# ErickRosete/tacorl

Measured on NVIDIA B200. Metric: play_lmp_train_frames_per_sec, higher is better.
Workload: dtype bf16

## Files before the change

tacorl_b200/csrc/gemm_tc.cu:

```cuda
#include "common.cuh"
#include "internal.h"
#include <cuda.h>
#include <cuda_bf16.h>
#include <algorithm>

namespace tacorl {

constexpr int TC_BM = 128;
constexpr int TC_BK = 64;
constexpr int TC_UMMA_K = 16;
constexpr int TC_THREADS = 192;

__device__ __forceinline__ uint32_t smem_u32(const void* p) { return (uint32_t)__cvta_generic_to_shared(p); }

__device__ __forceinline__ void mbar_init(uint32_t bar, uint32_t count) {
  asm volatile("mbarrier.init.shared::cta.b64 [%0], %1;" ::"r"(bar), "r"(count));
}
__device__ __forceinline__ void mbar_expect_tx(uint32_t bar, uint32_t bytes) {
  asm volatile("mbarrier.arrive.expect_tx.shared::cta.b64 _, [%0], %1;" ::"r"(bar), "r"(bytes) : "memory");
}
__device__ __forceinline__ void mbar_wait(uint32_t bar, uint32_t parity) {
  uint32_t done;
  do {
    asm volatile(
// ... 501 lines not shown
    for (int j = 0; j < 4; ++j) {
      if (ep.act == ACT_RELU) v[j] = fmaxf(v[j], 0.f);
      else if (ep.act == ACT_SILU) v[j] = v[j] / (1.f + __expf(-v[j]));
      if (g4[j] <= 0.f) v[j] = 0.f;
    }
    if (ep.C) *reinterpret_cast<float4*>(ep.C + (long long)b * ep.ldc + col) = make_float4(v[0], v[1], v[2], v[3]);
    if (ep.Cb) {
      __nv_bfloat162 lo = __floats2bfloat162_rn(v[0], v[1]), hi = __floats2bfloat162_rn(v[2], v[3]);
      uint2 pk = make_uint2(*reinterpret_cast<uint32_t*>(&lo), *reinterpret_cast<uint32_t*>(&hi));
      *reinterpret_cast<uint2*>(ep.Cb + (long long)b * ep.ldcb + col) = pk;
    }
  }
  RS_STAMP(9)
#ifdef RS_EXP_LATEARRIVE
  asm volatile("barrier.cluster.arrive.release.aligned;" ::: "memory");
#endif
  asm volatile("barrier.cluster.wait.aligned;" ::: "memory");
  RS_STAMP(10)
  RS_STAMP(11)
  RS_CTA_STAMP(1)
}

struct SeqArgs {
  int n_steps;
  int tau0, dtau;
  float beta;
  float* C; long long ldc, c_ts;
  const float* gate; long long ldgate, gate_ts;
  __nv_bfloat16* Cb; long long cb_ts;
  int act;
  unsigned* flags;
};
__device__ unsigned g_rnn_seq_timeouts = 0;
__device__ unsigned g_rnn_flags[2][32];
__device__ unsigned g_rnn_done = 0;
__device__ __forceinline__ void rnn_launch_epilogue(int tid) {
  if (tid == 0) {
    __threadfence();
    const unsigned total = gridDim.x * gridDim.y * gridDim.z;
    if (atomicAdd(&g_rnn_done, 1u) == total - 1) {
#pragma unroll
      for (int i = 0; i < 64; ++i) (&g_rnn_flags[0][0])[i] = 0;
      __threadfence();
      g_rnn_done = 0;
    }
  }
}
#ifdef TACORL_STEP_PROFILE
__device__ long long g_seq_prof[16];
#define SQ_STAMP(i) if (step == 8 && blockIdx.x == 1 && blockIdx.y == 3) g_seq_prof[i] = clock64();
#else
#define SQ_STAMP(i)
#endif

__device__ __forceinline__ void tma_load_3d(uint32_t dst, const CUtensorMap* tm, int c0, int c1, int c2, uint32_t bar) {
  asm volatile(
      "cp.async.bulk.tensor.3d.shared::cluster.global.mbarrier::complete_tx::bytes [%0], [%1, {%2, %3, %4}], [%5];"
      ::"r"(dst), "l"(tm), "r"(c0), "r"(c1), "r"(c2), "r"(bar) : "memory");
}
__device__ __forceinline__ unsigned ld_acquire_gpu(const unsigned* p) {
  unsigned v;
  asm volatile("ld.acquire.gpu.global.u32 %0, [%1];" : "=r"(v) : "l"(p) : "memory");
  return v;
}
__device__ __forceinline__ void red_release_gpu_add(unsigned* p, unsigned v) {
  asm volatile("red.release.gpu.global.add.u32 [%0], %1;" ::"l"(p), "r"(v) : "memory");
}

__global__ void __cluster_dims__(RS_KS, 1, 1) __launch_bounds__(RS_THREADS, 1)
rnn_seq_kernel(const __grid_constant__ CUtensorMap tmA, const __grid_constant__ CUtensorMap tmW, const SeqArgs sa,
               int M, int Mpad, int N, int NT, int kb_per_cta) {
  extern __shared__ __align__(1024) uint8_t smem_raw[];
  uint8_t* smem = (uint8_t*)(((uintptr_t)smem_raw + 1023) & ~(uintptr_t)1023);
  const uint32_t A_TILE = 128 * 128, W_BYTES = (uint32_t)NT * 128, W_STAGE = (W_BYTES + 1023) & ~1023u;
  const int SP = NT + 4;
  const int per = Mpad / RS_KS;
  uint8_t* w_smem = smem;
  uint8_t* a_smem = smem + (size_t)kb_per_cta * W_STAGE;
  float* S = (float*)(a_smem + (size_t)kb_per_cta * A_TILE);
  uint64_t* bars = (uint64_t*)((uint8_t*)S + (((size_t)((Mpad + 31) & ~31) * SP * 4 + 1023) & ~(size_t)1023));
  uint32_t* tmem_slot = (uint32_t*)(bars + 10);
  const int tid = threadIdx.x, warp = tid >> 5, lane = tid & 31;
  const uint32_t rank = blockIdx.x;
  const int tile = blockIdx.y, n0 = tile * NT, tiles = gridDim.y;
  const uint32_t tmem_cols = NT <= 32 ? 32 : (NT <= 64 ? 64 : (NT <= 128 ? 128 : 256));
  const uint32_t done_bar = smem_u32(bars + 8), w_bar = smem_u32(bars + 9);

  if (tid == RS_EPI) {
    for (int s = 0; s < kb_per_cta; ++s) mbar_init(smem_u32(bars + s), 1);
    mbar_init(done_bar, 1);
    mbar_init(w_bar, 1);
    asm volatile("fence.mbarrier_init.release.cluster;" ::: "memory");
  }
  if (warp == RS_EPI / 32) {
    asm volatile("tcgen05.alloc.cta_group::1.sync.aligned.shared::cta.b32 [%0], %1;"
                 ::"r"(smem_u32(tmem_slot)), "r"(tmem_cols) : "memory");
    asm volatile("tcgen05.relinquish_alloc_permit.cta_group::1.sync.aligned;" ::: "memory");
  }
  tc_fence_before();
  __syncthreads();
  tc_fence_after();
  const uint32_t tmem_base = *tmem_slot;
  const int k_begin = (int)rank * kb_per_cta * TC_BK;

  if (tid == RS_EPI) {
    mbar_expect_tx(w_bar, (uint32_t)kb_per_cta * W_BYTES);
    for (int s = 0; s < kb_per_cta; ++s)
      tma_load_2d(smem_u32(w_smem + (size_t)s * W_STAGE), &tmW, k_begin + s * TC_BK, n0, w_bar);
  }
  const int j_lo = k_begin / NT, j_hi = min(tiles - 1, (k_begin + kb_per_cta * TC_BK - 1) / NT);
  const int NT4 = NT >> 2, elems = per * NT4;
  bool dead = false;

  for (int step = 0; step < sa.n_steps; ++step) {
    const int tau = sa.tau0 + step * sa.dtau;
// ... 114 lines not shown
#pragma unroll
      for (int i = 0; i < RS_MAXE; ++i) dep += acc[i].x + acc[i].y + acc[i].z + acc[i].w;
      asm volatile("barrier.cluster.arrive.release.aligned;" ::"f"(dep) : "memory");
      if (tid == 0) { SQ_STAMP(8) }
      float* Ct = sa.C + (long long)tau * sa.c_ts;
      __nv_bfloat16* Bt = sa.Cb + (long long)tau * sa.cb_ts;
      float4 outv[RS_MAXE];
      bool okv[RS_MAXE];
#pragma unroll
      for (int i = 0; i < RS_MAXE; ++i) {
        const int e = tid + i * RS_EPI;
        const int bi = e / NT4, n = (e - bi * NT4) * 4, b = (int)rank * per + bi, col = n0 + n;
        okv[i] = e < elems && b < M && col < N;
        float v[4] = {acc[i].x, acc[i].y, acc[i].z, acc[i].w};
        const float c4[4] = {cold[i].x, cold[i].y, cold[i].z, cold[i].w};
        const float g4[4] = {gt[i].x, gt[i].y, gt[i].z, gt[i].w};
#pragma unroll
        for (int j = 0; j < 4; ++j) {
          v[j] = fmaf(sa.beta, c4[j], v[j]);
          if (sa.act == ACT_RELU) v[j] = fmaxf(v[j], 0.f);
          if (g4[j] <= 0.f) v[j] = 0.f;
        }
        outv[i] = make_float4(v[0], v[1], v[2], v[3]);
        if (okv[i]) {
          __nv_bfloat162 lo = __floats2bfloat162_rn(v[0], v[1]), hi = __floats2bfloat162_rn(v[2], v[3]);
          *reinterpret_cast<uint2*>(Bt + (long long)b * N + col) =
              make_uint2(*reinterpret_cast<uint32_t*>(&lo), *reinterpret_cast<uint32_t*>(&hi));
        }
      }
      asm volatile("fence.proxy.async.global;" ::: "memory");
      if (tid == 0) { SQ_STAMP(9) }
      asm volatile("bar.sync 1, %0;" ::"n"(RS_EPI) : "memory");
      if (tid == 0) { __threadfence(); red_release_gpu_add(&g_rnn_flags[0][tile], 1u); SQ_STAMP(10) }
#pragma unroll
      for (int i = 0; i < RS_MAXE; ++i) {
        const int e = tid + i * RS_EPI;
        const int bi = e / NT4, n = (e - bi * NT4) * 4, b = (int)rank * per + bi, col = n0 + n;
        if (okv[i]) *reinterpret_cast<float4*>(Ct + (long long)b * sa.ldc + col) = outv[i];
      }
    } else {
      asm volatile("barrier.cluster.arrive.release.aligned;" ::: "memory");
    }
  }
  asm volatile("barrier.cluster.wait.aligned;" ::: "memory");
  if (warp == RS_EPI / 32) {
    tc_fence_after();
    asm volatile("tcgen05.dealloc.cta_group::1.sync.aligned.b32 %0, %1;" ::"r"(tmem_base), "r"(tmem_cols) : "memory");
  }
  rnn_launch_epilogue(tid);
}

constexpr int RW_KS = 4;
constexpr int RW_MAX_TILES = 16;
struct WaveLane {
  int n_steps, tau0, dtau, act;
  float beta;
  float* C; long long ldc, c_ts;
  const float* gate; long long ldgate, gate_ts;
  __nv_bfloat16* Cb; long long ldcb, cb_ts;
  unsigned* flags;
};
struct WaveArgs { WaveLane lane[2]; };

__global__ void __launch_bounds__(RS_THREADS, 1)
rnn_wave_kernel(const __grid_constant__ CUtensorMap tmA0, const __grid_constant__ CUtensorMap tmW0,
                const __grid_constant__ CUtensorMap tmA1, const __grid_constant__ CUtensorMap tmW1,
                const __grid_constant__ WaveArgs wa, int M, int Mpad, int N, int NT, int kb_per_cta) {
  extern __shared__ __align__(1024) uint8_t smem_raw[];
  uint8_t* smem = (uint8_t*)(((uintptr_t)smem_raw + 1023) & ~(uintptr_t)1023);
  const uint32_t W_BYTES = (uint32_t)NT * 128, W_STAGE = (W_BYTES + 1023) & ~1023u, A_PITCH = (uint32_t)Mpad * 128;
  const int SP = NT + 4;
  const int per = Mpad / RW_KS;
  uint8_t* w_smem = smem;
  uint8_t* a_smem = smem + (size_t)kb_per_cta * W_STAGE;
  float* S = (float*)(a_smem + (size_t)kb_per_cta * A_PITCH);
  uint64_t* bars = (uint64_t*)((uint8_t*)S + (((size_t)((Mpad + 31) & ~31) * SP * 4 + 1023) & ~(size_t)1023));
  uint32_t* tmem_slot = (uint32_t*)(bars + 10);
  const int tid = threadIdx.x, warp = tid >> 5, lane = tid & 31;
  const uint32_t rank = blockIdx.x;
  const int tile = blockIdx.y, n0 = tile * NT, tiles = gridDim.y;
  const WaveLane& sa = wa.lane[blockIdx.z];
  const CUtensorMap* tmA = blockIdx.z ? &tmA1 : &tmA0;
  const CUtensorMap* tmW = blockIdx.z ? &tmW1 : &tmW0;
  const uint32_t tmem_cols = NT <= 32 ? 32 : (NT <= 64 ? 64 : 128);
  const uint32_t done_bar = smem_u32(bars + 8), w_bar = smem_u32(bars + 9);

  if (tid == RS_EPI) {
    for (int s = 0; s < kb_per_cta; ++s) mbar_init(smem_u32(bars + s), 1);
    mbar_init(done_bar, 1);
    mbar_init(w_bar, 1);
    asm volatile("fence.mbarrier_init.release.cluster;" ::: "memory");
  }
  if (warp == RS_EPI / 32) {
    asm volatile("tcgen05.alloc.cta_group::1.sync.aligned.shared::cta.b32 [%0], %1;"
                 ::"r"(smem_u32(tmem_slot)), "r"(tmem_cols) : "memory");
    asm volatile("tcgen05.relinquish_alloc_permit.cta_group::1.sync.aligned;" ::: "memory");
  }
  tc_fence_before();
  __syncthreads();
  tc_fence_after();
  const uint32_t tmem_base = *tmem_slot;
  const int k_begin = (int)rank * kb_per_cta * TC_BK;

  if (tid == RS_EPI) {
    mbar_expect_tx(w_bar, (uint32_t)kb_per_cta * W_BYTES);
    for (int s = 0; s < kb_per_cta; ++s)
      tma_load_2d(smem_u32(w_smem + (size_t)s * W_STAGE), tmW, k_begin + s * TC_BK, n0, w_bar);
  }
  const int j_lo = k_begin / NT, j_hi = min(tiles - 1, (k_begin + kb_per_cta * TC_BK - 1) / NT);
  const int NT4 = NT >> 2, elems = per * NT4;
  bool dead = false;

  for (int step = 0; step < sa.n_steps; ++step) {
    const int tau = sa.tau0 + step * sa.dtau;
    const uint32_t ph = (uint32_t)step & 1u;
    float4 cold[RS_MAXE], gt[RS_MAXE];
    if (warp == RS_EPI / 32) {
      if (step > 0 && !dead) {
        const unsigned want = (unsigned)(RW_KS * step);
        bool bad = false;
        for (int j = j_lo + lane; j <= j_hi; j += 32) {
          unsigned spins = 0;
          while (ld_acquire_gpu(&g_rnn_flags[blockIdx.z][j]) < want) {
            if (++spins > (1u << 21)) { bad = true; atomicAdd(&g_rnn_seq_timeouts, 1u); break; }
          }
        }
        if (__any_sync(0xffffffffu, bad)) dead = true;
        __threadfence();
        __syncwarp();
      }
      if (lane == 0) {
        if (step == 0) mbar_wait(w_bar, 0);
        asm volatile("fence.proxy.async.global;" ::: "memory");
        for (int s = 0; s < kb_per_cta; ++s) {
          const uint32_t bar = smem_u32(bars + s);
          mbar_expect_tx(bar, A_PITCH);
          tma_load_3d(smem_u32(a_smem + (size_t)s * A_PITCH), tmA, k_begin + s * TC_BK, 0, tau - sa.dtau, bar);
        }
        const uint32_t idesc = (1u << 4) | (1u << 7) | (1u << 10) | ((uint32_t)(NT >> 3) << 17) | ((uint32_t)(128 >> 4) << 24);
        for (int s = 0; s < kb_per_cta; ++s) {
          mbar_wait(smem_u32(bars + s), ph);
          tc_fence_after();
          const uint32_t a_src = smem_u32(a_smem + (size_t)s * A_PITCH), w_src = smem_u32(w_smem + (size_t)s * W_STAGE);
#pragma unroll
          for (int k = 0; k < TC_BK / TC_UMMA_K; ++k)
            tc_mma_bf16(tmem_base, make_smem_desc(a_src + k * 32, 16, 1024), make_smem_desc(w_src + k * 32, 16, 1024), idesc,
                        (s > 0 || k > 0) ? 1u : 0u);
        }
        tc_commit(done_bar);
      }
      __syncwarp();
    } else {
      const float* Ct = sa.C + (long long)tau * sa.c_ts;
      const float* Gt = sa.gate ? sa.gate + (long long)tau * sa.gate_ts : nullptr;
      long long offc[RS_MAXE], offg[RS_MAXE];
#pragma unroll
      for (int i = 0; i < RS_MAXE; ++i) {
        const int e = tid + i * RS_EPI;
        const int bi = e / NT4, n = (e - bi * NT4) * 4, b = (int)rank * per + bi, col = n0 + n;
        const bool ok = e < elems && b < M && col < N;
        offc[i] = ok ? (long long)b * sa.ldc + col : 0;
        offg[i] = ok ? (long long)b * sa.ldgate + col : 0;
      }
      const float4 zero = make_float4(0.f, 0.f, 0.f, 0.f), one = make_float4(1.f, 1.f, 1.f, 1.f);
#pragma unroll
      for (int i = 0; i < RS_MAXE; ++i) cold[i] = sa.beta != 0.f ? *reinterpret_cast<const float4*>(Ct + offc[i]) : zero;
#pragma unroll
      for (int i = 0; i < RS_MAXE; ++i) gt[i] = Gt ? *reinterpret_cast<const float4*>(Gt + offg[i]) : one;
      mbar_wait(done_bar, ph);
      tc_fence_after();
    }
    if (step > 0) asm volatile("barrier.cluster.wait.aligned;" ::: "memory");
    if (warp < RS_EPI / 32) {
      const int q = warp & 3;
      if (q * 32 < Mpad) {
        float* Srow = S + (q * 32 + lane) * SP;
        uint32_t r[2][16];
#pragma unroll
        for (int i = 0; i < 2; ++i) {
          const int c0 = (warp >> 2) * 16 + 64 * i;
          if (c0 < NT) tc_ld16_nowait(tmem_base + ((uint32_t)(q * 32) << 16) + c0, r[i]);
        }
        tc_ld_wait();
#pragma unroll
        for (int i = 0; i < 2; ++i) {
          const int c0 = (warp >> 2) * 16 + 64 * i;
          if (c0 < NT) {
#pragma unroll
            for (int j = 0; j < 4; ++j)
              reinterpret_cast<float4*>(Srow + c0)[j] = make_float4(__uint_as_float(r[i][4 * j]), __uint_as_float(r[i][4 * j + 1]),
                                                                    __uint_as_float(r[i][4 * j + 2]), __uint_as_float(r[i][4 * j + 3]));
          }
        }
      }
    }
    tc_fence_before();
    cluster_sync_all();
    tc_fence_after();
    float4 acc[RS_MAXE];
    if (warp < RS_EPI / 32) {
      float4 part[RS_MAXE][RW_KS];
#pragma unroll
      for (int i = 0; i < RS_MAXE; ++i) {
        const int e = tid + i * RS_EPI;
        const int bi = e / NT4, n = (e - bi * NT4) * 4;
        const uint32_t addr = smem_u32(S + ((int)rank * per + (e < elems ? bi : 0)) * SP + (e < elems ? n : 0));
#pragma unroll
        for (int q = 0; q < RW_KS; ++q) part[i][q] = ld_dsmem_v4(addr, (q + rank) & (RW_KS - 1));
      }
#pragma unroll
      for (int i = 0; i < RS_MAXE; ++i) {
        float4 v = make_float4(0.f, 0.f, 0.f, 0.f);
#pragma unroll
        for (int q = 0; q < RW_KS; ++q) { v.x += part[i][q].x; v.y += part[i][q].y; v.z += part[i][q].z; v.w += part[i][q].w; }
        acc[i] = v;
      }
      float dep = 0.f;
#pragma unroll
      for (int i = 0; i < RS_MAXE; ++i) dep += acc[i].x + acc[i].y + acc[i].z + acc[i].w;
      asm volatile("barrier.cluster.arrive.release.aligned;" ::"f"(dep) : "memory");
      float* Ct = sa.C + (long long)tau * sa.c_ts;
      __nv_bfloat16* Bt = sa.Cb + (long long)tau * sa.cb_ts;
      float4 outv[RS_MAXE];
      bool okv[RS_MAXE];
#pragma unroll
      for (int i = 0; i < RS_MAXE; ++i) {
        const int e = tid + i * RS_EPI;
        const int bi = e / NT4, n = (e - bi * NT4) * 4, b = (int)rank * per + bi, col = n0 + n;
        okv[i] = e < elems && b < M && col < N;
        float v[4] = {acc[i].x, acc[i].y, acc[i].z, acc[i].w};
        const float c4[4] = {cold[i].x, cold[i].y, cold[i].z, cold[i].w};
        const float g4[4] = {gt[i].x, gt[i].y, gt[i].z, gt[i].w};
#pragma unroll
        for (int j = 0; j < 4; ++j) {
          v[j] = fmaf(sa.beta, c4[j], v[j]);
          if (sa.act == ACT_RELU) v[j] = fmaxf(v[j], 0.f);
          if (g4[j] <= 0.f) v[j] = 0.f;
        }
        outv[i] = make_float4(v[0], v[1], v[2], v[3]);
        if (okv[i]) {
          __nv_bfloat162 lo = __floats2bfloat162_rn(v[0], v[1]), hi = __floats2bfloat162_rn(v[2], v[3]);
          *reinterpret_cast<uint2*>(Bt + (long long)b * sa.ldcb + col) =
              make_uint2(*reinterpret_cast<uint32_t*>(&lo), *reinterpret_cast<uint32_t*>(&hi));
        }
      }
      asm volatile("fence.proxy.async.global;" ::: "memory");
      asm volatile("bar.sync 1, %0;" ::"n"(RS_EPI) : "memory");
      if (tid == 0) { __threadfence(); red_release_gpu_add(&g_rnn_flags[blockIdx.z][tile], 1u); }
#pragma unroll
      for (int i = 0; i < RS_MAXE; ++i) {
        const int e = tid + i * RS_EPI;
        const int bi = e / NT4, n = (e - bi * NT4) * 4, b = (int)rank * per + bi, col = n0 + n;
        if (okv[i]) *reinterpret_cast<float4*>(Ct + (long long)b * sa.ldc + col) = outv[i];
      }
    } else {
      asm volatile("barrier.cluster.arrive.release.aligned;" ::: "memory");
    }
  }
  if (sa.n_steps > 0) asm volatile("barrier.cluster.wait.aligned;" ::: "memory");
  if (warp == RS_EPI / 32) {
    tc_fence_after();
    asm volatile("tcgen05.dealloc.cta_group::1.sync.aligned.b32 %0, %1;" ::"r"(tmem_base), "r"(tmem_cols) : "memory");
  }
  rnn_launch_epilogue(tid);
}

typedef CUresult (*EncodeTiledFn)(CUtensorMap*, CUtensorMapDataType, cuuint32_t, void*, const cuuint64_t*,
                                  const cuuint64_t*, const cuuint32_t*, const cuuint32_t*, CUtensorMapInterleave,
                                  CUtensorMapSwizzle, CUtensorMapL2promotion, CUtensorMapFloatOOBfill);

static EncodeTiledFn get_encode_fn() {
  static EncodeTiledFn fn = nullptr;
  if (!fn) {
    void* p = nullptr;
    cudaDriverEntryPointQueryResult q;
    if (cudaGetDriverEntryPoint("cuTensorMapEncodeTiled", &p, cudaEnableDefault, &q) == cudaSuccess &&
        q == cudaDriverEntryPointSuccess)
      fn = (EncodeTiledFn)p;
  }
  return fn;
}

static int make_tmap(CUtensorMap* tm, const void* base, long long inner, long long outer, long long ld,
                     int box_inner, int box_outer) {
  EncodeTiledFn fn = get_encode_fn();
  TACORL_REQUIRE(fn, "gemm_tc: cuTensorMapEncodeTiled is not available from the driver");
  TACORL_REQUIRE(((uintptr_t)base & 15) == 0 && (ld * 2) % 16 == 0,
                 "gemm_tc: TMA operand must be 16-byte aligned with a 16-byte multiple pitch (ld=%lld)", ld);
  cuuint64_t dims[2] = {(cuuint64_t)inner, (cuuint64_t)outer};
  cuuint64_t strides[1] = {(cuuint64_t)ld * 2};
  cuuint32_t box[2] = {(cuuint32_t)box_inner, (cuuint32_t)box_outer};
  cuuint32_t estr[2] = {1, 1};
  CUresult r = fn(tm, CU_TENSOR_MAP_DATA_TYPE_BFLOAT16, 2, const_cast<void*>(base), dims, strides, box, estr,
                  CU_TENSOR_MAP_INTERLEAVE_NONE, CU_TENSOR_MAP_SWIZZLE_128B, CU_TENSOR_MAP_L2_PROMOTION_L2_256B,
                  CU_TENSOR_MAP_FLOAT_OOB_FILL_NONE);
  TACORL_REQUIRE(r == CUDA_SUCCESS, "gemm_tc: cuTensorMapEncodeTiled failed (%d) inner=%lld outer=%lld ld=%lld", (int)r,
                 inner, outer, ld);
  return 0;
}

template <int BN, bool A_MN, bool B_MN>
static int launch_tc(const CUtensorMap& ta, const CUtensorMap& tb, const TcEpilogue& ep, int M, int N, int K,
                     int splits, cudaStream_t st) {
  constexpr int kStages = BN >= 128 ? 5 : 6;
  constexpr size_t smem = (size_t)kStages * (TC_BM * TC_BK * 2 + BN * TC_BK * 2) + (2 * kStages + 4) * 8 + 16 + 1024;
  static bool configured = false;
  auto kern = gemm_tc_kernel<BN, A_MN, B_MN, kStages>;
  if (!configured) {
    TACORL_CHECK_CUDA(cudaFuncSetAttribute(kern, cudaFuncAttributeMaxDynamicSharedMemorySize, (int)smem));
    configured = true;
  }
  const int total_kb = cdiv(K, TC_BK);
  const int per = cdiv(total_kb, splits);
  const int zs = cdiv(total_kb, per);
  const long long tiles = (long long)cdiv(N, BN) * cdiv(M, TC_BM);
// ... 110 lines not shown
  {
    static size_t checked_smem = 0;
    static int max_clusters = 0;
    if (checked_smem != smem) {
      cudaLaunchConfig_t cfg = {};
      cfg.gridDim = dim3(RS_KS, tiles); cfg.blockDim = dim3(RS_THREADS); cfg.dynamicSmemBytes = smem;
      cudaLaunchAttribute at[1];
      at[0].id = cudaLaunchAttributeClusterDimension;
      at[0].val.clusterDim.x = RS_KS; at[0].val.clusterDim.y = 1; at[0].val.clusterDim.z = 1;
      cfg.attrs = at; cfg.numAttrs = 1;
      int n = 0;
      if (cudaOccupancyMaxActiveClusters(&n, rnn_seq_kernel, &cfg) != cudaSuccess) { cudaGetLastError(); n = 0; }
      max_clusters = n; checked_smem = smem;
    }
    if (max_clusters < tiles) return 1;
  }
  CUtensorMap ta, tw;
  int rc;
  {
    EncodeTiledFn fn = get_encode_fn();
    TACORL_REQUIRE(fn, "rnn_seq: cuTensorMapEncodeTiled is not available from the driver");
    TACORL_REQUIRE(((uintptr_t)Ab & 15) == 0, "rnn_seq: hidden-state buffer must be 16-byte aligned");
    cuuint64_t dims[3] = {(cuuint64_t)K, (cuuint64_t)M, (cuuint64_t)T};
    cuuint64_t strides[2] = {(cuuint64_t)K * 2, (cuuint64_t)M * K * 2};
    cuuint32_t box[3] = {64, (cuuint32_t)Mpad, 1};
    cuuint32_t estr[3] = {1, 1, 1};
    CUresult r = fn(&ta, CU_TENSOR_MAP_DATA_TYPE_BFLOAT16, 3, const_cast<void*>(Ab), dims, strides, box, estr,
                    CU_TENSOR_MAP_INTERLEAVE_NONE, CU_TENSOR_MAP_SWIZZLE_128B, CU_TENSOR_MAP_L2_PROMOTION_L2_256B,
                    CU_TENSOR_MAP_FLOAT_OOB_FILL_NONE);
    TACORL_REQUIRE(r == CUDA_SUCCESS, "rnn_seq: cuTensorMapEncodeTiled failed (%d) K=%d M=%d T=%d", (int)r, K, M, T);
  }
  if ((rc = make_tmap(&tw, W, K, N, ldw, 64, NT))) return rc;
  SeqArgs sa;
  sa.n_steps = n_steps; sa.tau0 = tau0; sa.dtau = dtau; sa.beta = beta; sa.C = C; sa.ldc = ldc; sa.c_ts = c_ts;
  sa.gate = gate; sa.ldgate = ldgate; sa.gate_ts = gate_ts; sa.Cb = (__nv_bfloat16*)Cb; sa.cb_ts = (long long)M * N;
  sa.act = act; sa.flags = flags;
  int rc2;
  if ((rc2 = persistent_chain_enter(st))) return rc2;
  rnn_seq_kernel<<<dim3(RS_KS, tiles), RS_THREADS, smem, st>>>(ta, tw, sa, M, Mpad, N, NT, kb);
  TACORL_LAUNCH_CHECK();
  if ((rc2 = persistent_chain_leave(st))) return rc2;
  return 0;
}

int rnn_wave_tc(const WaveLaneHost* lanes, int n_lanes, int T, int M, int N, int K, cudaStream_t st) {
  if (!rnn_seq_enabled() || n_lanes < 1 || n_lanes > 2) return 1;
  if (n_lanes == 2 && rnn_seq_mode() == 2) {
    int rc = rnn_wave_tc(lanes, 1, T, M, N, K, st);
    return rc ? rc : rnn_wave_tc(lanes + 1, 1, T, M, N, K, st);
  }
  if (M < 1 || M > 64 || K != N || K % (TC_BK * RW_KS) != 0 || N % 4 != 0) return 1;
  const int Mpad = (M + 15) & ~15, kb = K / (TC_BK * RW_KS);
  const int NT = 16 * cdiv(N, 16 * RW_MAX_TILES), tiles = cdiv(N, NT);
  if (NT > 128 || kb > 8 || (Mpad / RW_KS) * (NT / 4) > RS_MAXE * RS_EPI) return 1;
  auto al16 = [](const void* p, long long ld) { return p == nullptr || (((uintptr_t)p & 15) == 0 && (ld * 4) % 16 == 0); };
  int max_steps = 0;
  for (int l = 0; l < n_lanes; ++l) {
    const WaveLaneHost& h = lanes[l];
    if (!h.Ab || !h.W || !h.C || !h.Cb || !h.flags || h.n_steps < 0) return 1;
    if (!al16(h.C, h.ldc) || !al16(h.C, h.c_ts) || !al16(h.gate, h.ldgate) || !al16(h.gate, h.gate_ts)) return 1;
    if (((uintptr_t)h.Cb & 7) != 0 || h.ldcb % 4 != 0 || h.cb_ts % 4 != 0) return 1;
    if (((uintptr_t)h.Ab & 15) != 0 || (h.lda * 2) % 16 != 0 || (h.a_ts * 2) % 16 != 0) return 1;
    max_steps = std::max(max_steps, h.n_steps);
  }
  if (max_steps < 2) return 1;
  const size_t w_stage = ((size_t)NT * 128 + 1023) & ~(size_t)1023, a_pitch = (size_t)Mpad * 128;
  const size_t s_bytes = ((size_t)((Mpad + 31) & ~31) * (NT + 4) * 4 + 1023) & ~(size_t)1023;
  const size_t tail = std::max(a_pitch + s_bytes + 256, (size_t)16384 + 256);
  const size_t smem = (size_t)kb * w_stage + (size_t)(kb - 1) * a_pitch + tail + 1024;
  if (smem > 227 * 1024) return 1;
  static size_t configured = 0;
  if (smem > configured) {
    TACORL_CHECK_CUDA(cudaFuncSetAttribute(rnn_wave_kernel, cudaFuncAttributeMaxDynamicSharedMemorySize, (int)smem));
    TACORL_CHECK_CUDA(cudaFuncSetAttribute(rnn_wave_kernel, cudaFuncAttributeNonPortableClusterSizeAllowed, 0));
    configured = smem;
  }
  cudaLaunchConfig_t cfg = {};
  cfg.gridDim = dim3(RW_KS, tiles, n_lanes); cfg.blockDim = dim3(RS_THREADS); cfg.dynamicSmemBytes = smem; cfg.stream = st;
  cudaLaunchAttribute at[1];
  at[0].id = cudaLaunchAttributeClusterDimension;
  at[0].val.clusterDim.x = RW_KS; at[0].val.clusterDim.y = 1; at[0].val.clusterDim.z = 1;
  cfg.attrs = at; cfg.numAttrs = 1;
  {
    static size_t checked_smem = 0;
    static int max_clusters = 0;
    if (checked_smem != smem) {
      int n = 0;
      if (cudaOccupancyMaxActiveClusters(&n, rnn_wave_kernel, &cfg) != cudaSuccess) { cudaGetLastError(); n = 0; }
      max_clusters = n; checked_smem = smem;
    }
    if (max_clusters < tiles * n_lanes) return 1;
  }
  EncodeTiledFn fn = get_encode_fn();
  TACORL_REQUIRE(fn, "rnn_wave: cuTensorMapEncodeTiled is not available from the driver");
  CUtensorMap ta[2], tw[2];
  WaveArgs wa;
  int rc;
  for (int l = 0; l < 2; ++l) {
    const WaveLaneHost& h = lanes[l < n_lanes ? l : 0];
    cuuint64_t dims[3] = {(cuuint64_t)K, (cuuint64_t)M, (cuuint64_t)T};
    cuuint64_t strides[2] = {(cuuint64_t)h.lda * 2, (cuuint64_t)h.a_ts * 2};
    cuuint32_t box[3] = {64, (cuuint32_t)Mpad, 1};
    cuuint32_t estr[3] = {1, 1, 1};
    CUresult r = fn(&ta[l], CU_TENSOR_MAP_DATA_TYPE_BFLOAT16, 3, const_cast<void*>(h.Ab), dims, strides, box, estr,
                    CU_TENSOR_MAP_INTERLEAVE_NONE, CU_TENSOR_MAP_SWIZZLE_128B, CU_TENSOR_MAP_L2_PROMOTION_L2_256B,
                    CU_TENSOR_MAP_FLOAT_OOB_FILL_NONE);
    TACORL_REQUIRE(r == CUDA_SUCCESS, "rnn_wave: cuTensorMapEncodeTiled failed (%d) K=%d M=%d T=%d", (int)r, K, M, T);
    if ((rc = make_tmap(&tw[l], h.W, K, N, h.ldw, 64, NT))) return rc;
    WaveLane& d = wa.lane[l];
    d.n_steps = l < n_lanes ? h.n_steps : 0; d.tau0 = h.tau0; d.dtau = h.dtau; d.act = h.act; d.beta = h.beta;
    d.C = h.C; d.ldc = h.ldc; d.c_ts = h.c_ts; d.gate = h.gate; d.ldgate = h.ldgate; d.gate_ts = h.gate_ts;
    d.Cb = (__nv_bfloat16*)h.Cb; d.ldcb = h.ldcb; d.cb_ts = h.cb_ts; d.flags = h.flags;
  }
  if ((rc = persistent_chain_enter(st))) return rc;
  void* args[] = {&ta[0], &tw[0], &ta[1], &tw[1], &wa, (void*)&M, (void*)&Mpad, (void*)&N, (void*)&NT, (void*)&kb};
  TACORL_CHECK_CUDA(cudaLaunchKernelExC(&cfg, (const void*)rnn_wave_kernel, args));
  note_launch();
  if ((rc = persistent_chain_leave(st))) return rc;
  return 0;
}

unsigned rnn_seq_timeouts() {
// ... 131 lines not shown
```

Baseline: 316,200.

## Restructure RNN wave kernel into warp-specialized pipeline with async DSMEM push reduction

```diff
diff --git a/tacorl_b200/csrc/gemm_tc.cu b/tacorl_b200/csrc/gemm_tc.cu
--- a/tacorl_b200/csrc/gemm_tc.cu
+++ b/tacorl_b200/csrc/gemm_tc.cu
@@ -577,6 +577,18 @@
 #else
 #define SQ_STAMP(i)
 #endif
+#ifdef TACORL_STEP_PROFILE
+__device__ long long g_wave_prof[16];
+#define WV_STAMP(i) if (step == 8 && blockIdx.x == 1 && blockIdx.y == 3 && blockIdx.z == 0) g_wave_prof[i] = clock64();
+#define WV_PERIOD() if (step == 9 && blockIdx.x == 1 && blockIdx.y == 3 && blockIdx.z == 0) g_wave_prof[15] = clock64();
+static const char* const kWaveStageNames[] = {
+    "issuer: step start", "issuer: tmem free", "issuer: flags ok, tma issued", "issuer: first h stage landed",
+    "issuer: mma issued+commit", "drain: mma done", "drain: tmem read", "drain: slot free", "drain: parts pushed",
+    "owner: peers' parts landed", "owner: summed, slots returned", "owner: bf16 stored, released"};
+#else
+#define WV_STAMP(i)
+#define WV_PERIOD()
+#endif
 
 __device__ __forceinline__ void tma_load_3d(uint32_t dst, const CUtensorMap* tm, int c0, int c1, int c2, uint32_t bar) {
   asm volatile(
@@ -586,6 +598,11 @@
 __device__ __forceinline__ unsigned ld_acquire_gpu(const unsigned* p) {
   unsigned v;
   asm volatile("ld.acquire.gpu.global.u32 %0, [%1];" : "=r"(v) : "l"(p) : "memory");
+  return v;
+}
+__device__ __forceinline__ unsigned ld_relaxed_gpu(const unsigned* p) {
+  unsigned v;
+  asm volatile("ld.relaxed.gpu.global.u32 %0, [%1];" : "=r"(v) : "l"(p) : "memory");
   return v;
 }
 __device__ __forceinline__ void red_release_gpu_add(unsigned* p, unsigned v) {
@@ -806,6 +823,7 @@
 
 constexpr int RW_KS = 4;
 constexpr int RW_MAX_TILES = 16;
+constexpr int RW_TMEM_COLS = 64;
 struct WaveLane {
   int n_steps, tau0, dtau, act;
   float beta;
@@ -816,6 +834,42 @@
 };
 struct WaveArgs { WaveLane lane[2]; };
 
+__device__ __forceinline__ uint32_t mapa_cta(uint32_t local_addr, uint32_t cta) {
+  uint32_t remote;
+  asm volatile("mapa.shared::cluster.u32 %0, %1, %2;" : "=r"(remote) : "r"(local_addr), "r"(cta));
+  return remote;
+}
+__device__ __forceinline__ void st_async_v4(uint32_t remote, uint32_t a, uint32_t b, uint32_t c, uint32_t d, uint32_t rbar) {
+  asm volatile("st.async.shared::cluster.mbarrier::complete_tx::bytes.v4.b32 [%0], {%1, %2, %3, %4}, [%5];"
+               ::"r"(remote), "r"(a), "r"(b), "r"(c), "r"(d), "r"(rbar) : "memory");
+}
+__device__ __forceinline__ void st_async_b32(uint32_t remote, uint32_t a, uint32_t rbar) {
+  asm volatile("st.async.shared::cluster.mbarrier::complete_tx::bytes.b32 [%0], %1, [%2];" ::"r"(remote), "r"(a), "r"(rbar)
+               : "memory");
+}
+__device__ __forceinline__ void mbar_arrive_remote(uint32_t rbar) {
+  asm volatile("mbarrier.arrive.release.cluster.shared::cluster.b64 _, [%0];" ::"r"(rbar) : "memory");
+}
+template <bool kCluster>
+__device__ __forceinline__ void mbar_wait_bounded(uint32_t bar, uint32_t parity, bool& dead) {
+  if (dead) return;
+  for (unsigned spins = 0;; ++spins) {
+    uint32_t done;
+    if (kCluster)
+      asm volatile("{\n\t.reg .pred p;\n\tmbarrier.try_wait.parity.acquire.cluster.shared::cta.b64 p, [%1], %2;\n\t"
+                   "selp.u32 %0, 1, 0, p;\n\t}" : "=r"(done) : "r"(bar), "r"(parity) : "memory");
+    else
+      asm volatile("{\n\t.reg .pred p;\n\tmbarrier.try_wait.parity.shared::cta.b64 p, [%1], %2;\n\t"
+                   "selp.u32 %0, 1, 0, p;\n\t}" : "=r"(done) : "r"(bar), "r"(parity) : "memory");
+    if (done) return;
+    if (spins > (1u << 20)) { dead = true; atomicAdd(&g_rnn_seq_timeouts, 1u); return; }
+  }
+}
+__device__ __forceinline__ void tc_ld4_nowait(uint32_t taddr, uint32_t (&r)[4]) {
+  asm volatile("tcgen05.ld.sync.aligned.32x32b.x4.b32 {%0,%1,%2,%3}, [%4];"
+               : "=r"(r[0]), "=r"(r[1]), "=r"(r[2]), "=r"(r[3]) : "r"(taddr));
+}
+
 __global__ void __launch_bounds__(RS_THREADS, 1)
 rnn_wave_kernel(const __grid_constant__ CUtensorMap tmA0, const __grid_constant__ CUtensorMap tmW0,
                 const __grid_constant__ CUtensorMap tmA1, const __grid_constant__ CUtensorMap tmW1,
@@ -823,198 +877,219 @@
   extern __shared__ __align__(1024) uint8_t smem_raw[];
   uint8_t* smem = (uint8_t*)(((uintptr_t)smem_raw + 1023) & ~(uintptr_t)1023);
   const uint32_t W_BYTES = (uint32_t)NT * 128, W_STAGE = (W_BYTES + 1023) & ~1023u, A_PITCH = (uint32_t)Mpad * 128;
-  const int SP = NT + 4;
-  const int per = Mpad / RW_KS;
+  const int per = Mpad / RW_KS, R = per / 4;
+  const int P = per + ((per & 4) ? 0 : 4);
   uint8_t* w_smem = smem;
   uint8_t* a_smem = smem + (size_t)kb_per_cta * W_STAGE;
-  float* S = (float*)(a_smem + (size_t)kb_per_cta * A_PITCH);
-  uint64_t* bars = (uint64_t*)((uint8_t*)S + (((size_t)((Mpad + 31) & ~31) * SP * 4 + 1023) & ~(size_t)1023));
-  uint32_t* tmem_slot = (uint32_t*)(bars + 10);
+  float* slot = (float*)(a_smem + (size_t)kb_per_cta * A_PITCH);
+  uint64_t* bars = (uint64_t*)(slot + 3 * 128 * P);
+  uint32_t* tmem_slot = (uint32_t*)(bars + 16);
   const int tid = threadIdx.x, warp = tid >> 5, lane = tid & 31;
   const uint32_t rank = blockIdx.x;
   const int tile = blockIdx.y, n0 = tile * NT, tiles = gridDim.y;
   const WaveLane& sa = wa.lane[blockIdx.z];
   const CUtensorMap* tmA = blockIdx.z ? &tmA1 : &tmA0;
   const CUtensorMap* tmW = blockIdx.z ? &tmW1 : &tmW0;
-  const uint32_t tmem_cols = NT <= 32 ? 32 : (NT <= 64 ? 64 : 128);
-  const uint32_t done_bar = smem_u32(bars + 8), w_bar = smem_u32(bars + 9);
+  const uint32_t done_bar = smem_u32(bars + 8), w_bar = smem_u32(bars + 9), full_bar = smem_u32(bars + 10),
+                 empty_bar = smem_u32(bars + 11), tmem_empty_bar = smem_u32(bars + 12);
 
   if (tid == RS_EPI) {
     for (int s = 0; s < kb_per_cta; ++s) mbar_init(smem_u32(bars + s), 1);
     mbar_init(done_bar, 1);
     mbar_init(w_bar, 1);
+    mbar_init(full_bar, 1);
+    mbar_init(empty_bar, (RW_KS - 1) * (RS_EPI / 32));
+    mbar_init(tmem_empty_bar, RS_EPI / 32);
     asm volatile("fence.mbarrier_init.release.cluster;" ::: "memory");
   }
   if (warp == RS_EPI / 32) {
     asm volatile("tcgen05.alloc.cta_group::1.sync.aligned.shared::cta.b32 [%0], %1;"
-                 ::"r"(smem_u32(tmem_slot)), "r"(tmem_cols) : "memory");
+                 ::"r"(smem_u32(tmem_slot)), "r"(RW_TMEM_COLS) : "memory");
     asm volatile("tcgen05.relinquish_alloc_permit.cta_group::1.sync.aligned;" ::: "memory");
   }
   tc_fence_before();
-  __syncthreads();
+  cluster_sync_all();
   tc_fence_after();
   const uint32_t tmem_base = *tmem_slot;
   const int k_begin = (int)rank * kb_per_cta * TC_BK;
-
-  if (tid == RS_EPI) {
-    mbar_expect_tx(w_bar, (uint32_t)kb_per_cta * W_BYTES);
-    for (int s = 0; s < kb_per_cta; ++s)
-      tma_load_2d(smem_u32(w_smem + (size_t)s * W_STAGE), tmW, k_begin + s * TC_BK, n0, w_bar);
-  }
-  const int j_lo = k_begin / NT, j_hi = min(tiles - 1, (k_begin + kb_per_cta * TC_BK - 1) / NT);
-  const int NT4 = NT >> 2, elems = per * NT4;
   bool dead = false;
 
-  for (int step = 0; step < sa.n_steps; ++step) {
-    const int tau = sa.tau0 + step * sa.dtau;
-    const uint32_t ph = (uint32_t)step & 1u;
-    float4 cold[RS_MAXE], gt[RS_MAXE];
-    if (warp == RS_EPI / 32) {
-      if (step > 0 && !dead) {
+  if (warp == RS_EPI / 32) {
+    if (lane == 0) {
+      mbar_expect_tx(w_bar, (uint32_t)kb_per_cta * W_BYTES);
+      for (int s = 0; s < kb_per_cta; ++s)
+        tma_load_2d(smem_u32(w_smem + (size_t)s * W_STAGE), tmW, k_begin + s * TC_BK, n0, w_bar);
+      const uint32_t idesc = (1u << 4) | (1u << 7) | (1u << 10) | ((uint32_t)(Mpad >> 3) << 17) | ((uint32_t)(128 >> 4) << 24);
+      for (int step = 0; step < sa.n_steps; ++step) {
+        const int tau = sa.tau0 + step * sa.dtau;
+        WV_STAMP(0) WV_PERIOD()
+        if (step > 0) { mbar_wait_bounded<false>(tmem_empty_bar, (uint32_t)(step - 1) & 1u, dead); tc_fence_after(); }
+        else mbar_wait(w_bar, 0);
+        WV_STAMP(1)
+#ifdef WV_EXP_CTA
         const unsigned want = (unsigned)(RW_KS * step);
-        bool bad = false;
-        for (int j = j_lo + lane; j <= j_hi; j += 32) {
-          unsigned spins = 0;
-          while (ld_acquire_gpu(&g_rnn_flags[blockIdx.z][j]) < want) {
-            if (++spins > (1u << 21)) { bad = true; atomicAdd(&g_rnn_seq_timeouts, 1u); break; }
+#else
+        const unsigned want = (unsigned)(RW_KS * (RS_EPI / 32) * step);
+#endif
+        const int j_hi = min(tiles - 1, (k_begin + kb_per_cta * TC_BK - 1) / NT);
+        int j_ready = step > 0 ? k_begin / NT - 1 : tiles;
+        for (int s = 0; s < kb_per_cta; ++s) {
+          const int k0 = k_begin + s * TC_BK, j_need = min(tiles - 1, (k0 + TC_BK - 1) / NT);
+#ifdef WV_EXP_PAR
+          if (j_ready < j_need) {
+            unsigned spins = 0;
+            while (!dead) {
+              unsigned v[4];
+#pragma unroll
+              for (int u = 0; u < 4; ++u)
+                v[u] = j_ready + 1 + u <= j_hi ? ld_relaxed_gpu(&g_rnn_flags[blockIdx.z][j_ready + 1 + u]) : 0u;
+              int pre = j_ready;
+#pragma unroll
+              for (int u = 0; u < 4; ++u)
+                if (pre == j_ready + u && j_ready + 1 + u <= j_hi && v[u] >= want) pre = j_ready + 1 + u;
+              j_ready = pre;
+              if (j_ready >= j_need) break;
+              if (++spins > (1u << 21)) { dead = true; atomicAdd(&g_rnn_seq_timeouts, 1u); }
+            }
+            asm volatile("fence.acq_rel.gpu;" ::: "memory");
+          }
+#else
+          for (; j_ready < j_need; ++j_ready) {
+            unsigned spins = 0;
+            while (!dead && ld_acquire_gpu(&g_rnn_flags[blockIdx.z][j_ready + 1]) < want)
+              if (++spins > (1u << 21)) { dead = true; atomicAdd(&g_rnn_seq_timeouts, 1u); }
+          }
+#endif
+          asm volatile("fence.proxy.async.global;" ::: "memory");
+          const uint32_t bar = smem_u32(bars + s);
+          mbar_expect_tx(bar, A_PITCH);
+          tma_load_3d(smem_u32(a_smem + (size_t)s * A_PITCH), tmA, k0, 0, tau - sa.dtau, bar);
+        }
+        WV_STAMP(2)
+        for (int s = 0; s < kb_per_cta; ++s) {
+          mbar_wait(smem_u32(bars + s), (uint32_t)step & 1u);
+          tc_fence_after();
+          if (s == 0) { WV_STAMP(3) }
+          const uint64_t ad = make_smem_desc(smem_u32(w_smem + (size_t)s * W_STAGE), 16, 1024);
+          const uint64_t bd = make_smem_desc(smem_u32(a_smem + (size_t)s * A_PITCH), 16, 1024);
+#pragma unroll
+          for (int k = 0; k < TC_BK / TC_UMMA_K; ++k)
+            tc_mma_bf16(tmem_base, ad + 2 * k, bd + 2 * k, idesc, (s > 0 || k > 0) ? 1u : 0u);
+        }
+        tc_commit(done_bar);
+        WV_STAMP(4)
+      }
+    }
+    __syncwarp();
+  } else {
+    const int q = warp & 3, g = warp >> 2, n = q * 32 + lane, col = n0 + n;
+    const uint32_t t_lane = tmem_base + ((uint32_t)(q * 32) << 16);
+    uint32_t dst[RW_KS - 1], dst_bar[RW_KS - 1];
+    const uint32_t my_off = (uint32_t)((n * P + g * R) * 4);
+#pragma unroll
+    for (int i = 0; i < RW_KS - 1; ++i) {
+      const uint32_t d = (rank + 1 + i) & (RW_KS - 1), j = (rank - d - 1) & (RW_KS - 1);
+      dst[i] = mapa_cta(smem_u32(slot) + j * 128 * P * 4 + my_off, d);
+      dst_bar[i] = mapa_cta(full_bar, d);
+    }
+    const uint32_t src_empty = mapa_cta(empty_bar, (rank + 1 + (uint32_t)min(lane, RW_KS - 2)) & (RW_KS - 1));
+    const uint32_t full_bytes = (uint32_t)((RW_KS - 1) * 128 * per * 4);
+    for (int step = 0; step < sa.n_steps; ++step) {
+      const int tau = sa.tau0 + step * sa.dtau;
+      const uint32_t ph = (uint32_t)step & 1u;
+      if (tid == 0) mbar_expect_tx(full_bar, full_bytes);
+      const float* Ct = sa.C + (long long)tau * sa.c_ts;
+      const float* Gt = sa.gate ? sa.gate + (long long)tau * sa.gate_ts : nullptr;
+      float cold[4], gt[4];
+      bool ok[4];
+#pragma unroll
+      for (int i = 0; i < 4; ++i) {
+        const int b = (int)rank * per + g * R + i;
+        ok[i] = i < R && b < M && n < NT && col < N;
+        cold[i] = ok[i] && sa.beta != 0.f ? Ct[(long long)b * sa.ldc + col] : 0.f;
+        gt[i] = ok[i] && Gt ? Gt[(long long)b * sa.ldgate + col] : 1.f;
+      }
+      mbar_wait(done_bar, ph);
+      tc_fence_after();
+      if (tid == 0) { WV_STAMP(5) }
+      uint32_t part[RW_KS][4];
+#pragma unroll
+      for (int i = 0; i < RW_KS; ++i)
+        tc_ld4_nowait(t_lane + ((rank + i) & (RW_KS - 1)) * per + g * R, part[i]);
+      tc_ld_wait();
+      tc_fence_before();
+      __syncwarp();
+      if (lane == 0) mbar_arrive(tmem_empty_bar);
+      if (tid == 0) { WV_STAMP(6) }
+      if (step > 0) mbar_wait_bounded<true>(empty_bar, ph ^ 1u, dead);
+      if (tid == 0) { WV_STAMP(7) }
+#pragma unroll
+      for (int i = 0; i < RW_KS - 1; ++i) {
+        if (R == 4) {
+          st_async_v4(dst[i], part[i + 1][0], part[i + 1][1], part[i + 1][2], part[i + 1][3], dst_bar[i]);
+        } else {
+#pragma unroll
+          for (int r = 0; r < 4; ++r)
+            if (r < R) st_async_b32(dst[i] + 4 * r, part[i + 1][r], dst_bar[i]);
+        }
+      }
+      if (tid == 0) { WV_STAMP(8) }
+      mbar_wait_bounded<false>(full_bar, ph, dead);
+      if (tid == 0) { WV_STAMP(9) }
+      float v[4];
+      {
+        float in[RW_KS - 1][4];
+        const float* my = slot + n * P + g * R;
+#pragma unroll
+        for (int j = 0; j < RW_KS - 1; ++j) {
+          if (R == 4) {
+            const float4 t = *reinterpret_cast<const float4*>(my + j * 128 * P);
+            in[j][0] = t.x; in[j][1] = t.y; in[j][2] = t.z; in[j][3] = t.w;
+          } else {
+#pragma unroll
+            for (int r = 0; r < 4; ++r) in[j][r] = r < R ? my[j * 128 * P + r] : 0.f;
           }
         }
-        if (__any_sync(0xffffffffu, bad)) dead = true;
-        __threadfence();
-        __syncwarp();
-      }
-      if (lane == 0) {
-        if (step == 0) mbar_wait(w_bar, 0);
-        asm volatile("fence.proxy.async.global;" ::: "memory");
-        for (int s = 0; s < kb_per_cta; ++s) {
-          const uint32_t bar = smem_u32(bars + s);
-          mbar_expect_tx(bar, A_PITCH);
-          tma_load_3d(smem_u32(a_smem + (size_t)s * A_PITCH), tmA, k_begin + s * TC_BK, 0, tau - sa.dtau, bar);
+#pragma unroll
+        for (int r = 0; r < 4; ++r) {
+          float acc = 0.f;
+          acc += __uint_as_float(part[0][r]);
+#pragma unroll
+          for (int j = 0; j < RW_KS - 1; ++j) acc += in[j][r];
+          v[r] = acc;
         }
-        const uint32_t idesc = (1u << 4) | (1u << 7) | (1u << 10) | ((uint32_t)(NT >> 3) << 17) | ((uint32_t)(128 >> 4) << 24);
-        for (int s = 0; s < kb_per_cta; ++s) {
-          mbar_wait(smem_u32(bars + s), ph);
-          tc_fence_after();
-          const uint32_t a_src = smem_u32(a_smem + (size_t)s * A_PITCH), w_src = smem_u32(w_smem + (size_t)s * W_STAGE);
-#pragma unroll
-          for (int k = 0; k < TC_BK / TC_UMMA_K; ++k)
-            tc_mma_bf16(tmem_base, make_smem_desc(a_src + k * 32, 16, 1024), make_smem_desc(w_src + k * 32, 16, 1024), idesc,
-                        (s > 0 || k > 0) ? 1u : 0u);
-        }
-        tc_commit(done_bar);
       }
       __syncwarp();
-    } else {
-      const float* Ct = sa.C + (long long)tau * sa.c_ts;
-      const float* Gt = sa.gate ? sa.gate + (long long)tau * sa.gate_ts : nullptr;
-      long long offc[RS_MAXE], offg[RS_MAXE];
-#pragma unroll
-      for (int i = 0; i < RS_MAXE; ++i) {
-        const int e = tid + i * RS_EPI;
-        const int bi = e / NT4, n = (e - bi * NT4) * 4, b = (int)rank * per + bi, col = n0 + n;
-        const bool ok = e < elems && b < M && col < N;
-        offc[i] = ok ? (long long)b * sa.ldc + col : 0;
-        offg[i] = ok ? (long long)b * sa.ldgate + col : 0;
-      }
-      const float4 zero = make_float4(0.f, 0.f, 0.f, 0.f), one = make_float4(1.f, 1.f, 1.f, 1.f);
-#pragma unroll
-      for (int i = 0; i < RS_MAXE; ++i) cold[i] = sa.beta != 0.f ? *reinterpret_cast<const float4*>(Ct + offc[i]) : zero;
-#pragma unroll
-      for (int i = 0; i < RS_MAXE; ++i) gt[i] = Gt ? *reinterpret_cast<const float4*>(Gt + offg[i]) : one;
-      mbar_wait(done_bar, ph);
-      tc_fence_after();
-    }
-    if (step > 0) asm volatile("barrier.cluster.wait.aligned;" ::: "memory");
-    if (warp < RS_EPI / 32) {
-      const int q = warp & 3;
-      if (q * 32 < Mpad) {
-        float* Srow = S + (q * 32 + lane) * SP;
-        uint32_t r[2][16];
-#pragma unroll
-        for (int i = 0; i < 2; ++i) {
-          const int c0 = (warp >> 2) * 16 + 64 * i;
-          if (c0 < NT) tc_ld16_nowait(tmem_base + ((uint32_t)(q * 32) << 16) + c0, r[i]);
-        }
-        tc_ld_wait();
-#pragma unroll
-        for (int i = 0; i < 2; ++i) {
-          const int c0 = (warp >> 2) * 16 + 64 * i;
-          if (c0 < NT) {
-#pragma unroll
-            for (int j = 0; j < 4; ++j)
-              reinterpret_cast<float4*>(Srow + c0)[j] = make_float4(__uint_as_float(r[i][4 * j]), __uint_as_float(r[i][4 * j + 1]),
-                                                                    __uint_as_float(r[i][4 * j + 2]), __uint_as_float(r[i][4 * j + 3]));
-          }
-        }
-      }
-    }
-    tc_fence_before();
-    cluster_sync_all();
-    tc_fence_after();
-    float4 acc[RS_MAXE];
-    if (warp < RS_EPI / 32) {
-      float4 part[RS_MAXE][RW_KS];
-#pragma unroll
-      for (int i = 0; i < RS_MAXE; ++i) {
-        const int e = tid + i * RS_EPI;
-        const int bi = e / NT4, n = (e - bi * NT4) * 4;
-        const uint32_t addr = smem_u32(S + ((int)rank * per + (e < elems ? bi : 0)) * SP + (e < elems ? n : 0));
-#pragma unroll
-        for (int q = 0; q < RW_KS; ++q) part[i][q] = ld_dsmem_v4(addr, (q + rank) & (RW_KS - 1));
-      }
-#pragma unroll
-      for (int i = 0; i < RS_MAXE; ++i) {
-        float4 v = make_float4(0.f, 0.f, 0.f, 0.f);
-#pragma unroll
-        for (int q = 0; q < RW_KS; ++q) { v.x += part[i][q].x; v.y += part[i][q].y; v.z += part[i][q].z; v.w += part[i][q].w; }
-        acc[i] = v;
-      }
-      float dep = 0.f;
-#pragma unroll
-      for (int i = 0; i < RS_MAXE; ++i) dep += acc[i].x + acc[i].y + acc[i].z + acc[i].w;
-      asm volatile("barrier.cluster.arrive.release.aligned;" ::"f"(dep) : "memory");
-      float* Ct = sa.C + (long long)tau * sa.c_ts;
+      if (lane < RW_KS - 1) mbar_arrive_remote(src_empty);
+      if (tid == 0) { WV_STAMP(10) }
+      float* Cw = sa.C + (long long)tau * sa.c_ts;
       __nv_bfloat16* Bt = sa.Cb + (long long)tau * sa.cb_ts;
-      float4 outv[RS_MAXE];
-      bool okv[RS_MAXE];
-#pragma unroll
-      for (int i = 0; i < RS_MAXE; ++i) {
-        const int e = tid + i * RS_EPI;
-        const int bi = e / NT4, n = (e - bi * NT4) * 4, b = (int)rank * per + bi, col = n0 + n;
-        okv[i] = e < elems && b < M && col < N;
-        float v[4] = {acc[i].x, acc[i].y, acc[i].z, acc[i].w};
-        const float c4[4] = {cold[i].x, cold[i].y, cold[i].z, cold[i].w};
-        const float g4[4] = {gt[i].x, gt[i].y, gt[i].z, gt[i].w};
-#pragma unroll
-        for (int j = 0; j < 4; ++j) {
-          v[j] = fmaf(sa.beta, c4[j], v[j]);
-          if (sa.act == ACT_RELU) v[j] = fmaxf(v[j], 0.f);
-          if (g4[j] <= 0.f) v[j] = 0.f;
-        }
-        outv[i] = make_float4(v[0], v[1], v[2], v[3]);
-        if (okv[i]) {
-          __nv_bfloat162 lo = __floats2bfloat162_rn(v[0], v[1]), hi = __floats2bfloat162_rn(v[2], v[3]);
-          *reinterpret_cast<uint2*>(Bt + (long long)b * sa.ldcb + col) =
-              make_uint2(*reinterpret_cast<uint32_t*>(&lo), *reinterpret_cast<uint32_t*>(&hi));
-        }
+#pragma unroll
+      for (int i = 0; i < 4; ++i) {
+        v[i] = fmaf(sa.beta, cold[i], v[i]);
+        if (sa.act == ACT_RELU) v[i] = fmaxf(v[i], 0.f);
+        if (gt[i] <= 0.f) v[i] = 0.f;
+        if (ok[i]) Bt[(long long)((int)rank * per + g * R + i) * sa.ldcb + col] = __float2bfloat16(v[i]);
       }
       asm volatile("fence.proxy.async.global;" ::: "memory");
+#ifdef WV_EXP_CTA
       asm volatile("bar.sync 1, %0;" ::"n"(RS_EPI) : "memory");
-      if (tid == 0) { __threadfence(); red_release_gpu_add(&g_rnn_flags[blockIdx.z][tile], 1u); }
-#pragma unroll
-      for (int i = 0; i < RS_MAXE; ++i) {
-        const int e = tid + i * RS_EPI;
-        const int bi = e / NT4, n = (e - bi * NT4) * 4, b = (int)rank * per + bi, col = n0 + n;
-        if (okv[i]) *reinterpret_cast<float4*>(Ct + (long long)b * sa.ldc + col) = outv[i];
-      }
-    } else {
-      asm volatile("barrier.cluster.arrive.release.aligned;" ::: "memory");
-    }
-  }
-  if (sa.n_steps > 0) asm volatile("barrier.cluster.wait.aligned;" ::: "memory");
+      if (tid == 0) red_release_gpu_add(&g_rnn_flags[blockIdx.z][tile], 1u);
+#else
+      __syncwarp();
+      if (lane == 0) red_release_gpu_add(&g_rnn_flags[blockIdx.z][tile], 1u);
+#endif
+      if (tid == 0) { WV_STAMP(11) }
+#pragma unroll
+      for (int i = 0; i < 4; ++i)
+        if (ok[i]) Cw[(long long)((int)rank * per + g * R + i) * sa.ldc + col] = v[i];
+    }
+  }
+  tc_fence_before();
+  cluster_sync_all();
   if (warp == RS_EPI / 32) {
     tc_fence_after();
-    asm volatile("tcgen05.dealloc.cta_group::1.sync.aligned.b32 %0, %1;" ::"r"(tmem_base), "r"(tmem_cols) : "memory");
+    asm volatile("tcgen05.dealloc.cta_group::1.sync.aligned.b32 %0, %1;" ::"r"(tmem_base), "r"(RW_TMEM_COLS) : "memory");
   }
   rnn_launch_epilogue(tid);
 }
@@ -1231,7 +1306,7 @@
   if (M < 1 || M > 64 || K != N || K % (TC_BK * RW_KS) != 0 || N % 4 != 0) return 1;
   const int Mpad = (M + 15) & ~15, kb = K / (TC_BK * RW_KS);
   const int NT = 16 * cdiv(N, 16 * RW_MAX_TILES), tiles = cdiv(N, NT);
-  if (NT > 128 || kb > 8 || (Mpad / RW_KS) * (NT / 4) > RS_MAXE * RS_EPI) return 1;
+  if (NT > 128 || kb > 8) return 1;
   auto al16 = [](const void* p, long long ld) { return p == nullptr || (((uintptr_t)p & 15) == 0 && (ld * 4) % 16 == 0); };
   int max_steps = 0;
   for (int l = 0; l < n_lanes; ++l) {
@@ -1244,9 +1319,9 @@
   }
   if (max_steps < 2) return 1;
   const size_t w_stage = ((size_t)NT * 128 + 1023) & ~(size_t)1023, a_pitch = (size_t)Mpad * 128;
-  const size_t s_bytes = ((size_t)((Mpad + 31) & ~31) * (NT + 4) * 4 + 1023) & ~(size_t)1023;
-  const size_t tail = std::max(a_pitch + s_bytes + 256, (size_t)16384 + 256);
-  const size_t smem = (size_t)kb * w_stage + (size_t)(kb - 1) * a_pitch + tail + 1024;
+  const int per = Mpad / RW_KS, P = per + ((per & 4) ? 0 : 4);
+  const size_t layout = (size_t)kb * (w_stage + a_pitch) + (size_t)(RW_KS - 1) * 128 * P * 4 + 16 * 8 + 16;
+  const size_t smem = std::max(layout, (size_t)(kb - 1) * w_stage + 16384) + 1024;
   if (smem > 227 * 1024) return 1;
   static size_t configured = 0;
   if (smem > configured) {
```

Result: slower. 312,300 (median of 6 runs) (-1.2%).
